# NVIDIA/recsys-examples

Measured on AMD Instinct MI355X. Metric: embedding lookups/sec (DynamicEmb lookup+pool fwd+bwd, steady state), higher is better.
Workload: dtype f32 table rows, f32 accumulate, bf16 pooled output / gradients

## Files before the change

### recsys-examples_amd/csrc/hstu_attn.hip

```cpp
#include "common.h"
#include "../../include/recsys_amd.h"
#include <stdlib.h>
#include <type_traits>


#ifndef HSTU_F16
#define HSTU_F16 0
#endif
#if HSTU_F16
#define HSTU_FN(name) name##_f16
#define HSTU_NS_BEGIN namespace mi355 { inline namespace hstu_f16 {
#define HSTU_NS_END } }
#else
#define HSTU_FN(name) name
#define HSTU_NS_BEGIN namespace mi355 {
#define HSTU_NS_END }
#endif

HSTU_NS_BEGIN

#if HSTU_F16
typedef __attribute__((ext_vector_type(8))) _Float16 bf16x8_t;
#define HSTU_MFMA __builtin_amdgcn_mfma_f32_32x32x16_f16
#else
// ... 1548 lines not shown
  }
  __device__ __forceinline__ void commit_tr(uint16_t* dst, int row0, int L) const {
#pragma unroll
    for (int i = 0; i < PT; ++i) {
      const int ch = threadIdx.x + 256 * i;
      const u32x4_t z = {0u, 0u, 0u, 0u};
      const u32x4_t v = (row0 + ch / (D / 8) < L) ? r[i] : z;
      if (NCH % 256 == 0 || ch < NCH) *reinterpret_cast<u32x4_t*>(dst + (ch / (D / 8)) * TrStride<D>::value + 8 * (ch % (D / 8))) = v;
    }
  }
};

template <int D>
__device__ __forceinline__ void load_own_frags(bf16x8_t (&f)[D / 16], const uint16_t* base, int64_t row_stride, int row, int L, int hi) {
  const uint16_t* p = base + (int64_t)(row < L ? row : L - 1) * row_stride + 8 * hi;
#pragma unroll
  for (int sl = 0; sl < D / 16; ++sl) {
    const u32x4_t t = *reinterpret_cast<const u32x4_t*>(p + 16 * sl);
    f[sl] = __builtin_bit_cast(bf16x8_t, t);
  }
}

struct BwdAttnArgs {
  AttnArgs f;
  const uint16_t* dout; int64_t do_row, do_head;
  uint16_t* dq; uint16_t* dk; uint16_t* dv;
  uint16_t* ds_ws;
  uint16_t* p_ws;
  int ng;
  int bq_kv;
  const int64_t* plan_base;
  const int32_t* plan_chunk;
  int chunk;
  int tri;
  uint16_t* drab; int64_t drab_b, drab_h, drab_r;
  const int2* func_kvis; int64_t func_kvis_h;
  const int4* func_gext;
  int dq_row, dq_head, dk_row, dk_head, dv_row, dv_head;
};
struct XchUnit { int64_t base; int ngb; int tri; };
__device__ __forceinline__ XchUnit xch_unit(const BwdAttnArgs& g, int b, int h, int L) {
  XchUnit u;
  if (g.plan_base) { u.base = g.plan_base[b * g.f.H + h]; u.ngb = (L + 31) >> 5; u.tri = g.tri; }
  else { u.base = ((int64_t)b * g.f.H + h) * g.ng * g.ng; u.ngb = g.ng; u.tri = 0; }
  return u;
}
__device__ __forceinline__ int64_t xch_tile(const XchUnit& u, int kg, int qg) {
  return (u.base + (u.tri ? (int64_t)qg * (qg + 1) / 2 + kg : (int64_t)kg * u.ngb + qg)) * 1024;
}
__device__ __forceinline__ bool xch_absent(const XchUnit& u, int kg, int qg) { return u.tri && kg > qg; }
__device__ __forceinline__ bool xch_other_chunk(const BwdAttnArgs& g, int b, int h) {
  return g.plan_chunk != nullptr && g.plan_chunk[b * g.f.H + h] != g.chunk;
}
constexpr int kPlanMaxU = 4096;
constexpr int kPlanMaxChunks = 2048;
struct PlanView {
  const int64_t* F; int U;
  __device__ __forceinline__ int L(int64_t x) const {
    int lo = 0, hi = U;
    while (lo < hi) { const int mid = (lo + hi + 1) >> 1; if (F[mid] <= x) lo = mid; else hi = mid - 1; }
    return lo;
  }
  __device__ __forceinline__ int next(int s, int64_t c) const {
    const int64_t fs = F[s];
    const int z = L(fs), e = L(fs + c);
    return e > z ? e : (z + 1 < U ? z + 1 : U);
  }
  __device__ __forceinline__ int count(int64_t c) const {
    int n = 0;
    for (int s = 0; s < U; s = next(s, c)) ++n;
    return n > 0 ? n : 1;
  }
};
__global__ void __launch_bounds__(256) hstu_bwd_plan_kernel(const int* cu, int B, int H, int64_t cap_tiles, int tri, int64_t* base,
                                                            int32_t* chunk, int32_t* nchunks_out, int host_chunks, int* host_err) {
  __shared__ int64_t s_F[kPlanMaxU + 1];
  __shared__ int64_t s_part[256];
  __shared__ int s_start[kPlanMaxChunks + 1];
  __shared__ int64_t s_umax;
  __shared__ int s_n;
  __shared__ int64_t s_c;
  if (blockIdx.x != 0) return;
  const int tid = threadIdx.x;
  const int64_t U64 = (int64_t)B * H;
  const bool staged = U64 <= kPlanMaxU;
  if (staged) {
    const int U = (int)U64;
    const int per = (U + 255) / 256, u0 = tid * per < U ? tid * per : U, u1 = u0 + per < U ? u0 + per : U;
    int64_t sum = 0, mx = 1;
    {
      int b = u0 / H, h = u0 - b * H;
      int64_t nd = 0;
      for (int u = u0; u < u1; ++u) {
        if (u == u0 || h == 0) { const int64_t n = (cu[b + 1] - cu[b] + 31) >> 5; nd = tri ? n * (n + 1) / 2 : n * n; }
        s_F[u] = nd;
        sum += nd;
        mx = nd > mx ? nd : mx;
        if (++h == H) { h = 0; ++b; }
      }
    }
    s_part[tid] = sum;
    if (tid == 0) s_umax = 1;
    __syncthreads();
    atomicMax((unsigned long long*)&s_umax, (unsigned long long)mx);
    if (tid < 64) {
      int64_t v[4], run = 0;
// ... 1001 lines not shown
        const uint32_t drop = r0 + 1 < L ? 0u : 0xffffffffu;
        dma16(reinterpret_cast<const char*>(g + (int64_t)rc * row_stride), voff[u] - (rowterm & drop), d0 + u * 1024);
      }
    }
  }
};
typedef Dma64T<8> Dma64;
__device__ __forceinline__ bf16x8_t tr_frag_sw(const uint16_t* tile, int dt, int ks, int lane, int hi) {
  typedef short v4s_t __attribute__((ext_vector_type(4)));
  typedef short v8s_t __attribute__((ext_vector_type(8)));
  typedef __attribute__((address_space(3))) v4s_t* lds_v4s_t;
  const int il = lane & 15, g1 = (lane >> 4) & 1, vq = il >> 2;
  const uint16_t* p0 = tile + (16 * ks + 4 * hi + vq) * 256 + 4 * (il & 1) + 8 * (4 * (dt ^ vq) + 2 * g1 + ((il & 3) >> 1));
  const v4s_t lo4 = __builtin_amdgcn_ds_read_tr16_b64_v4i16((lds_v4s_t)(p0));
  const v4s_t hi4 = __builtin_amdgcn_ds_read_tr16_b64_v4i16((lds_v4s_t)(p0 + 8 * 256));
  const v8s_t r = {lo4.x, lo4.y, lo4.z, lo4.w, hi4.x, hi4.y, hi4.z, hi4.w};
  return __builtin_bit_cast(bf16x8_t, r);
}
template <int BUF>
__device__ __forceinline__ void gemm_x8(f32x16_t (&acc)[8], const uint16_t* ring, const bf16x8_t (&bf)[4], int lane, int hi) {
  constexpr int NB = 8, NVB = HSTU_X8_VBUF;
  const uint16_t* tile = ring + BUF * 64 * 256;
  bf16x8_t fr[NVB][4];
  auto load = [&](int bi) {
#pragma unroll
    for (int u = 0; u < 4; ++u) fr[bi % NVB][u] = tr_frag_sw(tile, 4 * (bi & 1) + u, bi >> 1, lane, hi);
  };
#pragma unroll
  for (int bi = 0; bi < NVB - 1; ++bi) load(bi);
#pragma unroll
  for (int bi = 0; bi < NB; ++bi) {
    if (bi + NVB - 1 < NB) load(bi + NVB - 1);
    __builtin_amdgcn_sched_barrier(0);
#pragma unroll
    for (int u = 0; u < 4; ++u) mfma_a(acc[4 * (bi & 1) + u], fr[bi % NVB][u], bf[bi >> 1]);
    __builtin_amdgcn_sched_barrier(0);
  }
}
template <int D>
__device__ __forceinline__ void store_acc_rows(const f32x16_t (&acc)[D / 32], uint16_t* rowp, int hi) {
#pragma unroll
  for (int dt = 0; dt < D / 32; ++dt)
#pragma unroll
    for (int g4 = 0; g4 < 4; ++g4) {
      uint2 o;
      o.x = pack_bf16(acc[dt][4 * g4 + 0], acc[dt][4 * g4 + 1]);
      o.y = pack_bf16(acc[dt][4 * g4 + 2], acc[dt][4 * g4 + 3]);
      *reinterpret_cast<uint2*>(rowp + 32 * dt + 8 * g4 + 4 * hi) = o;
    }
}

constexpr int kNW8 = 4;

template <int D, bool kFunc = false>
__device__ __forceinline__ void hstu_bwd_v_p8_body(const BwdAttnArgs& g, unsigned bz, unsigned nz) {
  constexpr int NW = kNW8, kBM8 = 32 * NW;
  static_assert(D == 256, "DMA rows of 32 chunks");
  const AttnArgs& a = g.f;
  constexpr int BQ = 64, NT = 2, TILE = BQ * D;
  extern __shared__ __attribute__((aligned(16))) uint16_t smem[];
  const BlockSeq bs = seq_head_of_block(a, bz, nz);
  const int b = bs.b, h = bs.h;
  SeqInfo s;
  s.start = bs.start;
  s.L = bs.end - s.start;
  const int n0 = bs.z * kBM8;
  if (n0 >= s.L || xch_other_chunk(g, b, h)) return;
  const XchUnit xu = xch_unit(g, b, h, s.L);
  s.has_ctx = a.num_contexts != nullptr;
  s.has_tgt = a.num_targets != nullptr;
  s.c = s.has_ctx ? a.num_contexts[b] : 0;
  s.hlen = s.L - (s.has_tgt ? a.num_targets[b] : 0);
  s.wl = a.wl; s.wr = a.wr;
  const int lane = lane_id(), hi = lane >> 5, l31 = lane & 31;
  const int wv = __builtin_amdgcn_readfirstlane((int)(threadIdx.x >> 6));
  const int key0 = n0 + 32 * wv, kj = key0 + l31;
  const bool wave_live = key0 < s.L;
  const uint16_t* dobase = g.dout + (int64_t)s.start * g.do_row + (int64_t)h * g.do_head;
  f32x16_t acc[D / 32];
#pragma unroll
  for (int dt = 0; dt < D / 32; ++dt)
#pragma unroll
    for (int r = 0; r < 16; ++r) acc[dt][r] = 0.f;
  static_assert(kBM8 == kBM, "one key block of the dK pass per workgroup");
  KvSpan sp = kv_span(a, s, n0, g.bq_kv);
  if constexpr (kFunc) sp = kv_span_clip(sp, func_kvis_of(g, s.start, b, h, n0), g.bq_kv);
  const int jump = sp.jump, c_end = sp.c_end, lim = sp.lim;
  const int jump_s = (jump / BQ) * BQ, cend_s = ((c_end + BQ - 1) / BQ) * BQ;
  int i_lim = ((lim + g.bq_kv - 1) / g.bq_kv) * g.bq_kv;
  if (i_lim > s.L) i_lim = s.L;
  auto advance = [&](int i) { i += BQ; return (i >= cend_s && i < jump_s) ? jump_s : i; };
  auto visited = [&](int i) { return i < s.L && kv_visited(sp, (i / g.bq_kv) * g.bq_kv); };
  Dma64T<NW> dma;
  dma.init(wv, lane, g.do_row);
  u32x4_t pn0[NT], pn1[NT];
  auto fetch_p = [&](int i) {
#pragma unroll
    for (int t = 0; t < NT; ++t) {
      const int it = i + 32 * t;
      if (wave_live && visited(it) && !xch_absent(xu, key0 >> 5, it >> 5)) {
        const u32x4_t* tp = reinterpret_cast<const u32x4_t*>(g.p_ws + xch_tile(xu, key0 >> 5, it >> 5)) + 2 * lane;
        pn0[t] = xch_load(tp); pn1[t] = xch_load(tp + 1);
      } else {
        pn0[t] = u32x4_t{0u, 0u, 0u, 0u}; pn1[t] = u32x4_t{0u, 0u, 0u, 0u};
      }
    }
  };
  int i0 = c_end > 0 ? 0 : jump_s;
  if (i0 < i_lim) { dma.issue(dobase, g.do_row, i0, s.L, smem, lane); fetch_p(i0); }
  auto step = [&](auto bufc) {
    constexpr int BUF = decltype(bufc)::value;
    bf16x8_t pf[2 * NT];
    asm volatile("s_waitcnt vmcnt(0)" ::: "memory");
#pragma unroll
    for (int t = 0; t < NT; ++t) { pf[2 * t] = __builtin_bit_cast(bf16x8_t, pn0[t]); pf[2 * t + 1] = __builtin_bit_cast(bf16x8_t, pn1[t]); }
    __syncthreads();
    {
      const int nx = advance(i0);
      if (nx < i_lim) { dma.issue(dobase, g.do_row, nx, s.L, smem + (BUF ^ 1) * TILE, lane); fetch_p(nx); }
    }
    if (wave_live) gemm_x8<BUF>(acc, smem, pf, lane, hi);
    i0 = advance(i0);
  };
  while (i0 < i_lim) {
    step(std::integral_constant<int, 0>{});
    if (i0 >= i_lim) break;
    step(std::integral_constant<int, 1>{});
  }
  asm volatile("s_waitcnt vmcnt(0)" ::: "memory");
  if (kj < s.L) store_acc_rows<D>(acc, g.dv + (int64_t)(s.start + kj) * g.dv_row + (int64_t)h * g.dv_head, hi);
}

template <int D, bool kFunc = false>
__device__ __forceinline__ void hstu_bwd_q_ds8_body(const BwdAttnArgs& g, unsigned bz, unsigned nz) {
  constexpr int NW = kNW8, kBM8 = 32 * NW;
  static_assert(D == 256, "DMA rows of 32 chunks");
  const AttnArgs& a = g.f;
  constexpr int BK = 64, NT = 2, TILE = BK * D;
  extern __shared__ __attribute__((aligned(16))) uint16_t smem[];
  const BlockSeq bs = seq_head_of_block(a, bz, nz);
  const int b = bs.b, h = bs.h;
  SeqInfo s;
  s.start = bs.start;
  s.L = bs.end - s.start;
  const int nblk = (s.L + kBM8 - 1) / kBM8;
  if (bs.z >= nblk || xch_other_chunk(g, b, h)) return;
  const XchUnit xu = xch_unit(g, b, h, s.L);
  const int m0 = row_block_of_rank(bs.z, nblk, a, b) * kBM8;
  s.has_ctx = a.num_contexts != nullptr;
  s.has_tgt = a.num_targets != nullptr;
  s.c = s.has_ctx ? a.num_contexts[b] : 0;
  s.hlen = s.L - (s.has_tgt ? a.num_targets[b] : 0);
  s.wl = a.wl; s.wr = a.wr;
  const int lane = lane_id(), hi = lane >> 5, l31 = lane & 31;
  const int wv = __builtin_amdgcn_readfirstlane((int)(threadIdx.x >> 6));
  uint16_t* dSw = smem + 2 * TILE + NT * 1024 * wv;
  const int qrow0 = m0 + 32 * wv, qi = qrow0 + l31;
  const bool wave_live = qrow0 < s.L;
  int last_row = m0 + kBM8 - 1 < s.L - 1 ? m0 + kBM8 - 1 : s.L - 1;
  int n_end = s.L;
  if (a.causal) { n_end = last_row + 1; if (s.has_ctx && m0 < s.c && s.hlen > n_end) n_end = s.hlen; }
  int w_last = qrow0 + 31 < s.L - 1 ? qrow0 + 31 : s.L - 1;
  int w_end = s.L;
  if (a.causal) { w_end = w_last + 1; if (s.has_ctx && qrow0 < s.c && s.hlen > w_end) w_end = s.hlen; }
  n_end = band_key_end(a, last_row, n_end);
  w_end = band_key_end(a, w_last, w_end);
  int n_beg = band_key_begin(a, m0, BK), w_beg = band_key_begin(a, qrow0, BK);
  const int it_kv = (qrow0 / g.bq_kv) * g.bq_kv;
  int2 vis_all = make_int2(0, 0x7fffffff);
  int gap_a = 0x7fffffff, gap_b = 0x7fffffff;
  int wgap_a = 0x7fffffff, wgap_b = 0x7fffffff;
  if constexpr (kFunc) {
    if (kBM * lane < s.L) vis_all = func_kvis_of(g, s.start, b, h, kBM * lane);
    if (g.func_gext && a.wskip) {
      FuncExt bx{0, 0x7fffffff, 0, 0x7fffffff}, wx = bx;
#pragma unroll
      for (int w = 0; w < NW; ++w) {
        const int row = m0 + 32 * w;
        const int64_t gi = func_gext_index(s.start, b, row);
        FuncExt e{0x7fffffff, 0, 0x7fffffff, 0};
        if (row >= s.L) e = FuncExt{0, 0x7fffffff, 0, 0x7fffffff};
        else if (gi < 4 * g.func_kvis_h) { const int4 t = g.func_gext[(int64_t)(a.func_h ? h : 0) * 4 * g.func_kvis_h + gi]; e = FuncExt{t.y, t.z, t.w, t.x}; }
        bx = func_ext_merge(bx, e);
        if (w == wv) wx = e;
      }
      const int be = func_ext_end(bx), bb = func_ext_begin(bx), we = func_ext_end(wx), wb = func_ext_begin(wx);
      if (be < n_end) n_end = be;
      if (we < w_end) w_end = we;
      if (bb > n_beg) n_beg = bb >= n_end ? n_end : (bb / BK) * BK;
      if (wb > w_beg) w_beg = wb >= 0x7fffff00 ? 0x7fffff00 : (wb / BK) * BK;
      if (bx.lo < bx.hi && bx.lo > bx.f0) {
        const int ga = ((bx.f0 + BK - 1) / BK) * BK, gb = (bx.lo / BK) * BK;
        if (ga < gb) { gap_a = ga; gap_b = gb; }
      }
      if (wx.lo < wx.hi && wx.lo > wx.f0) {
        const int ga = ((wx.f0 + BK - 1) / BK) * BK, gb = (wx.lo / BK) * BK;
        if (ga < gb) { wgap_a = ga; wgap_b = gb; }
      }
      if (n_beg >= gap_a && n_beg < gap_b) n_beg = gap_b;
    }
  }
  auto next_step = [&](int n) { n += BK; if constexpr (kFunc) { if (n >= gap_a && n < gap_b) n = gap_b; } return n; };
  f32x16_t acc[D / 32];
#pragma unroll
  for (int dt = 0; dt < D / 32; ++dt)
#pragma unroll
    for (int r = 0; r < 16; ++r) acc[dt][r] = 0.f;
  const uint16_t* kbase = a.k + (int64_t)s.start * a.k_row + (int64_t)h * a.k_head;
// ... 16 lines not shown
      sp = kv_span_clip(sp, vis, g.bq_kv);
    }
    return kv_visited(sp, it_kv);
  };
  auto fetch_ds = [&](int n) {
#pragma unroll
    for (int t = 0; t < NT; ++t) {
      const int nt = n + 32 * t;
      if (wave_live && nt < w_end && tile_written(nt) && !xch_absent(xu, nt >> 5, qrow0 >> 5)) {
        const u32x4_t* tp = reinterpret_cast<const u32x4_t*>(g.ds_ws + xch_tile(xu, nt >> 5, qrow0 >> 5)) + 2 * lane;
        ds0[t] = xch_load(tp); ds1[t] = xch_load(tp + 1);
      } else {
        ds0[t] = u32x4_t{0u, 0u, 0u, 0u}; ds1[t] = u32x4_t{0u, 0u, 0u, 0u};
      }
    }
  };
  if (n_end > n_beg) { dma.issue(kbase, a.k_row, n_beg, s.L, smem, lane); fetch_ds(n_beg); }
  int n0 = n_beg;
  auto step = [&](auto bufc) {
    constexpr int BUF = decltype(bufc)::value;
    asm volatile("s_waitcnt vmcnt(0)" ::: "memory");
#pragma unroll
    for (int t = 0; t < NT; ++t) {
      *reinterpret_cast<u32x4_t*>(dSw + 1024 * t + 16 * lane) = ds0[t];
      *reinterpret_cast<u32x4_t*>(dSw + 1024 * t + 16 * lane + 8) = ds1[t];
    }
    __syncthreads();
    { const int nx = next_step(n0); if (nx < n_end) { dma.issue(kbase, a.k_row, nx, s.L, smem + (BUF ^ 1) * TILE, lane); fetch_ds(nx); } }
    if (wave_live && n0 < w_end && n0 >= w_beg && !(kFunc && n0 >= wgap_a && n0 < wgap_b)) {
      bf16x8_t sf[2 * NT];
#pragma unroll
      for (int t = 0; t < NT; ++t)
#pragma unroll
        for (int half = 0; half < 2; ++half) {
          const uint16_t* pp = dSw + 1024 * t + tr_lane_off;
          const v4s_t lo4 = __builtin_amdgcn_ds_read_tr16_b64_v4i16((lds_v4s_t)(pp + (8 * (2 * half)) * 16));
          const v4s_t hi4 = __builtin_amdgcn_ds_read_tr16_b64_v4i16((lds_v4s_t)(pp + (8 * (2 * half + 1)) * 16));
          const v8s_t r = {lo4.x, lo4.y, lo4.z, lo4.w, hi4.x, hi4.y, hi4.z, hi4.w};
          sf[2 * t + half] = __builtin_bit_cast(bf16x8_t, r);
        }
      gemm_x8<BUF>(acc, smem, sf, lane, hi);
    }
    n0 = next_step(n0);
  };
  while (n0 < n_end) {
    step(std::integral_constant<int, 0>{});
    if (n0 >= n_end) break;
    step(std::integral_constant<int, 1>{});
  }
  asm volatile("s_waitcnt vmcnt(0)" ::: "memory");
  if (qi < s.L) store_acc_rows<D>(acc, g.dq + (int64_t)(s.start + qi) * g.dq_row + (int64_t)h * g.dq_head, hi);
}

template <int D, bool kFunc = false>
__global__ void __launch_bounds__(64 * kNW8, 2) hstu_bwd_vq8_kernel(BwdAttnArgs g) {
  const unsigned nz = gridDim.z >> 1;
  if (blockIdx.z < nz) hstu_bwd_v_p8_body<D, kFunc>(g, blockIdx.z, nz);
  else hstu_bwd_q_ds8_body<D, kFunc>(g, blockIdx.z - nz, nz);
}

template <int D, bool kFunc = false>
__global__ void __launch_bounds__(512) hstu_bwd_kv_pc_kernel(BwdAttnArgs g) {
  static_assert(D == 256, "DMA rows of 32 chunks");
  const AttnArgs& a = g.f;
  constexpr int BQ = 32, IMG = BQ * D;
  extern __shared__ __attribute__((aligned(16))) uint16_t smem[];
  uint16_t* const Qr = smem;
  uint16_t* const dOr = smem + 2 * IMG;
  uint16_t* const Qt = smem + 4 * IMG;
  uint16_t* const Hs = smem + 6 * IMG;
  int* const Fs = reinterpret_cast<int*>(smem + 6 * IMG + 2 * 4 * 2 * 64 * 8);

  const BlockSeq bs = seq_head_of_block(a);
  const int b = bs.b, h = bs.h;
  SeqInfo s;
  s.start = bs.start;
  s.L = bs.end - s.start;
  const int n0 = bs.z * kBM;
  if (n0 >= s.L || xch_other_chunk(g, b, h)) return;
  const XchUnit xu = xch_unit(g, b, h, s.L);
  s.has_ctx = a.num_contexts != nullptr;
  s.has_tgt = a.num_targets != nullptr;
  s.c = s.has_ctx ? a.num_contexts[b] : 0;
  s.hlen = s.L - (s.has_tgt ? a.num_targets[b] : 0);
  s.wl = a.wl; s.wr = a.wr;
  const int lane = lane_id(), hi = lane >> 5, l31 = lane & 31;
  const int wv = __builtin_amdgcn_readfirstlane((int)(threadIdx.x >> 6));
  const int role = wv >> 2, pw = wv & 3;
  const int key0 = n0 + 32 * pw, kj = key0 + l31;
  const bool wave_live = key0 < s.L;
  const bool plain = !s.has_ctx && !s.has_tgt && s.wl < 0 && s.wr < 0;
  const bool key_in = kj < s.L, key_hist = kj < s.hlen;
  const int key_iend = (s.has_tgt && kj >= s.hlen) ? s.hlen + ((kj - s.hlen) / a.group + 1) * a.group : 0x7fffffff;
  const int ctx_end = s.has_ctx ? s.c : 0;
  const uint16_t* qbase = a.q + (int64_t)s.start * a.q_row + (int64_t)h * a.q_head;
  const uint16_t* dobase = g.dout + (int64_t)s.start * g.do_row + (int64_t)h * g.do_head;
  const float neg_alpha_log2e = -a.alpha * 1.4426950408889634f;
  const float c_p = a.alpha * a.inv_scale, c_ds = a.alpha * a.inv_scale;
  KvSpan span = kv_span(a, s, n0, BQ);
  if constexpr (kFunc) span = kv_span_clip(span, func_kvis_of(g, s.start, b, h, n0), BQ);
  const int jump = span.jump, c_end = span.c_end, i_lim = span.lim;
  auto advance = [&](int i) { i += BQ; return (i >= c_end && i < jump) ? jump : i; };
  const int first = c_end > 0 ? 0 : jump;
#if HSTU_TIMING
  unsigned tsum[7] = {0, 0, 0, 0, 0, 0, 0};
  const unsigned t_start = tick();
  auto t_dump = [&]() {
    const unsigned t_end = tick();
    if (lane == 0) {
      const int blk = ((int)blockIdx.z * gridDim.y + blockIdx.y) * gridDim.x + blockIdx.x;
      unsigned long long* d = g_hstu_dbg + ((size_t)(blk * 8 + wv) % 65536) * 8;
      for (int i = 0; i < 7; ++i) d[i] = tsum[i];
      d[6] |= (unsigned long long)role << 32;
      d[7] = t_end - t_start;
    }
  };
#endif

  const int dr = lane >> 5, dp = lane & 31;
  uint32_t vq_k[4], vdo_k[4], vq_v[4];
#pragma unroll
  for (int u = 0; u < 4; ++u) {
    const int r = 2 * (4 * pw + u) + dr;
    vq_k[u] = (uint32_t)dr * (uint32_t)a.q_row * 2u + 16u * (uint32_t)(dp ^ (r & 15));
    vdo_k[u] = (uint32_t)dr * (uint32_t)g.do_row * 2u + 16u * (uint32_t)(dp ^ (r & 15));
    vq_v[u] = (uint32_t)dr * (uint32_t)a.q_row * 2u + 16u * (uint32_t)(dp ^ ((r & 3) << 2));
  }
  auto issue_img = [&](const uint16_t* gsrc, int64_t row_stride, const uint32_t (&voff)[4], int row0, uint16_t* dst) {
    const uint32_t d0 = __builtin_amdgcn_readfirstlane((uint32_t)(uintptr_t)(lds_void_t)(dst + 8 * pw * D));
    if (row0 + BQ <= s.L) {
      const char* sb = reinterpret_cast<const char*>(gsrc + (int64_t)(row0 + 8 * pw) * row_stride);
      const int64_t step = 2 * row_stride * 2;
#pragma unroll
      for (int u = 0; u < 4; ++u) Dma64::dma16(sb + u * step, voff[u], d0 + u * 1024);
    } else {
      const uint32_t rowterm = (uint32_t)dr * (uint32_t)row_stride * 2u;
#pragma unroll
      for (int u = 0; u < 4; ++u) {
        const int r0 = row0 + 2 * (4 * pw + u);
        const int rc = r0 < s.L ? r0 : s.L - 1;
        const uint32_t drop = r0 + 1 < s.L ? 0u : 0xffffffffu;
        Dma64::dma16(reinterpret_cast<const char*>(gsrc + (int64_t)rc * row_stride), voff[u] - (rowterm & drop), d0 + u * 1024);
      }
    }
  };

  if (role == 0) {
    bf16x8_t kf[D / 16], vf[D / 16];
    load_own_frags<D>(kf, a.k + (int64_t)s.start * a.k_row + (int64_t)h * a.k_head, a.k_row, kj, s.L, hi);
    load_own_frags<D>(vf, a.v + (int64_t)s.start * a.v_row + (int64_t)h * a.v_head, a.v_row, kj, s.L, hi);
    const int kx = l31 & 15;
    int cur = first, prev_valid = 0;
    auto step = [&](auto parc) {
      constexpr int PAR = decltype(parc)::value;
      TICK(t0);
      __syncthreads();
      TICK(t1);
      TACC(0, t0, t1);
      const int i0 = cur;
      const bool have = i0 < i_lim;
      prev_valid = have;
      cur = have ? advance(i0) : i0;
      if (!have || !wave_live) return;
// ... 162 lines not shown
        issue_img(dobase, g.do_row, vdo_k, nxt, dOr + (PAR ^ 1) * IMG);
        fetch_func(nxt);
      }
      issue_img(qbase, a.q_row, vq_v, i0, Qt + PAR * IMG);
    }
    prev_valid = have;
    cur = nxt;
    TICK(t3);
    TACC(2, t2, t3);
    if (!had || !wave_live) return;
    const u32x4_t* hp = reinterpret_cast<const u32x4_t*>(Hs) + (((PAR ^ 1) * 4 + pw) * 2) * 64 + lane;
    bf16x8_t sf[2];
    const u32x4_t y0 = hp[0], y1 = hp[64];
    sf[0] = __builtin_bit_cast(bf16x8_t, y0);
    sf[1] = __builtin_bit_cast(bf16x8_t, y1);
    if (ip < s.L && !xch_absent(xu, key0 >> 5, ip >> 5)) {
      u32x4_t* tq = reinterpret_cast<u32x4_t*>(g.ds_ws + xch_tile(xu, key0 >> 5, ip >> 5)) + 2 * lane;
      xch_store(tq, y0); xch_store(tq + 1, y1);
    }
    const uint16_t* tile = Qt + (PAR ^ 1) * IMG;
    constexpr int NB = 4;
    bf16x8_t fr[2][4];
    auto load = [&](int bi) {
#pragma unroll
      for (int u = 0; u < 4; ++u) fr[bi & 1][u] = tr_frag_sw(tile, 4 * (bi & 1) + u, bi >> 1, lane, hi);
    };
    load(0);
#pragma unroll
    for (int bi = 0; bi < NB; ++bi) {
      if (bi + 1 < NB) load(bi + 1);
      __builtin_amdgcn_sched_barrier(0);
#pragma unroll
      for (int u = 0; u < 4; ++u) mfma_a(acc_dk[4 * (bi & 1) + u], fr[bi & 1][u], sf[bi >> 1]);
      __builtin_amdgcn_sched_barrier(0);
    }
    TICK(t4);
    TACC(5, t3, t4);
#if HSTU_TIMING
    tsum[6] += 1;
#endif
  };
  while (cur < i_lim || prev_valid) {
    step(std::integral_constant<int, 0>{});
    if (!(cur < i_lim || prev_valid)) break;
    step(std::integral_constant<int, 1>{});
  }
  asm volatile("s_waitcnt vmcnt(0)" ::: "memory");
#if HSTU_TIMING
  t_dump();
#endif
  if (kj < s.L) store_acc_rows<D>(acc_dk, g.dk + (int64_t)(s.start + kj) * g.dk_row + (int64_t)h * g.dk_head, hi);
}


static int fwd_hook() {
  static const int v = getenv("MI355_HSTU_FWD") ? atoi(getenv("MI355_HSTU_FWD")) : 0;
  return v;
}

template <auto K, typename Args>
static int launch(dim3 grid, dim3 block, size_t smem, hipStream_t stream, const Args& args) {
  static bool attr_set = false;
  if (!attr_set) {
    const hipError_t e = hipFuncSetAttribute(reinterpret_cast<const void*>(K), hipFuncAttributeMaxDynamicSharedMemorySize, (int)smem);
    if (e != hipSuccess) { mi355_set_error(hipGetErrorString(e)); return MI355_ELAUNCH; }
    attr_set = true;
  }
  hipLaunchKernelGGL(K, grid, block, smem, stream, args);
  return MI355_OK;
}
static int launched(int failed) {
  if (failed) return MI355_ELAUNCH;
  MI355_LAUNCH_CHECK();
  return MI355_OK;
}

template <int D, int BQ, int MODE, bool kPre, bool kXP = false, bool kRab = false, bool kDq = false, bool kBoth = false>
static int launch_bwd_kv(const BwdAttnArgs& g, dim3 grid, hipStream_t stream) {
  constexpr bool kDV = MODE != 2, kDK = MODE != 1;
  const size_t timg = (size_t)BQ * TrStride<D>::value;
  const size_t smem = (size_t)(BQ * (D + 8) + (kDK ? BQ * (D + 8) + timg : 0) + (kDV ? timg : 0)) * sizeof(uint16_t);
  return launch<hstu_bwd_kv_kernel<D, BQ, MODE, kPre, kXP, kRab, kDq, kBoth>>(grid, dim3(256), smem, stream, g);
}
template <int D, int BK, bool kPre, bool kRab = false, bool kDq = false, bool kBoth = false>
static int launch_bwd_q(const BwdAttnArgs& g, dim3 grid, hipStream_t stream) {
  const size_t smem_q = (size_t)(2 * BK * (D + 8) + BK * TrStride<D>::value) * sizeof(uint16_t);
  return launch<hstu_bwd_q_kernel<D, BK, kPre, kRab, kDq, kBoth>>(grid, dim3(256), smem_q, stream, g);
}

template <int D>
static int launch_bwd_v_p(const BwdAttnArgs& g, dim3 grid, hipStream_t stream) {
  const size_t smem = (size_t)(HSTU_XSTEP * TrStride<D>::value) * sizeof(uint16_t);
  return launch<hstu_bwd_v_p_kernel<D>>(grid, dim3(256), smem, stream, g);
}

template <int D>
static int launch_bwd_q_ds(const BwdAttnArgs& g, dim3 grid, hipStream_t stream) {
  const size_t smem = (size_t)(HSTU_XSTEP * TrStride<D>::value + 4 * (HSTU_XSTEP / 32) * 1024) * sizeof(uint16_t);
  return launch<hstu_bwd_q_ds_kernel<D>>(grid, dim3(256), smem, stream, g);
}

template <bool kFunc>
static int launch_bwd_pc_x8(const BwdAttnArgs& g, dim3 grid, int B, int max_seqlen, hipStream_t stream) {
  const size_t smem_pc = (size_t)(6 * 32 * 256 + 2 * 4 * 2 * 64 * 8) * sizeof(uint16_t) + (kFunc ? 2 * 192 * sizeof(int) : 0);
  const size_t smem = (size_t)(2 * 64 * 256 + kNW8 * 2 * 1024) * sizeof(uint16_t);
  const int nblk = (max_seqlen + 32 * kNW8 - 1) / (32 * kNW8);
  return launched(launch<hstu_bwd_kv_pc_kernel<256, kFunc>>(grid, dim3(512), smem_pc, stream, g) ||
                  launch<hstu_bwd_vq8_kernel<256, kFunc>>(dim3(g.f.H, B, 2 * nblk), dim3(64 * kNW8), smem, stream, g));
}

template <int D>
static int launch_bwd(BwdAttnArgs g, int B, int max_seqlen, hipStream_t stream) {
  dim3 grid(g.f.H, B, (max_seqlen + kBM - 1) / kBM);
  if constexpr (D == 256) {
    if (g.f.func && !g.f.rab && g.f.n_func <= 5 && g.p_ws && g.ds_ws) {
      g.bq_kv = 32;
      return launch_bwd_pc_x8<true>(g, grid, B, max_seqlen, stream);
    }
  }
  if (g.f.rab && g.f.func) {
    g.ds_ws = g.p_ws = nullptr;
    g.bq_kv = 64;
    if constexpr (D >= 128)
      return launched(launch_bwd_kv<D, 64, 1, false, false, true, false, true>(g, grid, stream) ||
                      launch_bwd_kv<D, 32, 2, false, false, true, false, true>(g, grid, stream) ||
                      launch_bwd_q<D, D >= 256 ? 32 : 64, false, true, false, true>(g, grid, stream));
    else
      return launched(launch_bwd_kv<D, 64, 0, false, false, true, false, true>(g, grid, stream) ||
                      launch_bwd_q<D, 64, false, true, false, true>(g, grid, stream));
  }
  if (g.f.rab || g.f.func) {
    g.ds_ws = g.p_ws = nullptr;
    g.bq_kv = 64;
    if constexpr (D >= 128)
      return launched(launch_bwd_kv<D, 64, 1, false, false, true>(g, grid, stream) ||
                      launch_bwd_kv<D, 32, 2, false, false, true>(g, grid, stream) ||
                      launch_bwd_q<D, D >= 256 ? 32 : 64, false, true>(g, grid, stream));
    else
      return launched(launch_bwd_kv<D, 64, 0, false, false, true>(g, grid, stream) || launch_bwd_q<D, 64, false, true>(g, grid, stream));
  }
  if constexpr (D >= 256) {
    if (g.p_ws) {
      g.bq_kv = 32;
      return launch_bwd_pc_x8<false>(g, grid, B, max_seqlen, stream);
    }
    g.bq_kv = 64;
    return launched(launch_bwd_kv<D, 64, 1, true>(g, grid, stream) || launch_bwd_kv<D, 64, 2, false>(g, grid, stream) ||
                    (g.ds_ws ? launch_bwd_q_ds<D>(g, grid, stream) : launch_bwd_q<D, 32, true>(g, grid, stream)));
  } else if constexpr (D >= 128) {
    g.bq_kv = 32;
    if (g.p_ws)
      return launched(launch_bwd_kv<D, 32, 2, false, true>(g, grid, stream) || launch_bwd_v_p<D>(g, grid, stream) ||
                      launch_bwd_q_ds<D>(g, grid, stream));
    return launched(launch_bwd_kv<D, 64, 1, false>(g, grid, stream) || launch_bwd_kv<D, 32, 2, false>(g, grid, stream) ||
                    (g.ds_ws ? launch_bwd_q_ds<D>(g, grid, stream) : launch_bwd_q<D, 64, false>(g, grid, stream)));
  } else {
    g.bq_kv = 64;
    g.p_ws = nullptr;
    return launched(launch_bwd_kv<D, 64, 0, false>(g, grid, stream) ||
                    (g.ds_ws ? launch_bwd_q_ds<D>(g, grid, stream) : launch_bwd_q<D, 64, false>(g, grid, stream)));
  }
}

template <int D, bool kRab>
static int launch_bwd_dq(BwdAttnArgs g, int B, int max_q, int max_k, hipStream_t stream) {
  const dim3 gk(g.f.H, B, (max_k + kBM - 1) / kBM), gq(g.f.H, B, (max_q + kBM - 1) / kBM);
  g.ds_ws = g.p_ws = nullptr;
  g.bq_kv = 64;
  constexpr bool kPre = D >= 256 && !kRab;
  int failed;
  if constexpr (D >= 128)
    failed = launch_bwd_kv<D, 64, 1, kPre, false, kRab, true>(g, gk, stream) ||
             launch_bwd_kv<D, (D >= 256 && !kRab) ? 64 : 32, 2, false, false, kRab, true>(g, gk, stream);
  else
    failed = launch_bwd_kv<D, 64, 0, false, false, kRab, true>(g, gk, stream);
  return launched(failed || (max_q > 0 && launch_bwd_q<D, D >= 256 ? 32 : 64, kPre, kRab, true>(g, gq, stream)));
}

template <int D>
static int launch_fwd_pc(const AttnArgs& a, int B, int max_seqlen, hipStream_t stream, bool dense_batch) {
  const size_t smem = (size_t)(4 * kBN * D + 2 * 4 * 4 * 64 * 8) * sizeof(uint16_t);
  const int hook = fwd_hook();
  const bool paired = hook == 2 || hook == 4 || dense_batch;
  const bool q2 = hook == 1 || hook == 2 || (hook != 3 && hook != 4 && max_seqlen > 1024) || a.func;
  const int nblk = (max_seqlen + kBM - 1) / kBM;
  const bool win = a.wl >= 0 || a.wr >= 0;
  const dim3 grid(a.H, B, paired ? (nblk + 1) / 2 : nblk), block(512);
  if (q2) {
    if (a.func)
      return launched(paired ? launch<hstu_fwd_q2_kernel<D, true, true, true>>(grid, block, smem, stream, a)
                             : launch<hstu_fwd_q2_kernel<D, true, false, true>>(grid, block, smem, stream, a));
    if (paired)
      return launched(win ? launch<hstu_fwd_q2_kernel<D, true, true>>(grid, block, smem, stream, a)
                          : launch<hstu_fwd_q2_kernel<D, false, true>>(grid, block, smem, stream, a));
    return launched(win ? launch<hstu_fwd_q2_kernel<D, true, false>>(grid, block, smem, stream, a)
                        : launch<hstu_fwd_q2_kernel<D, false, false>>(grid, block, smem, stream, a));
  }
// ... 183 lines not shown
  if (batch == 0 || max_seqlen == 0) return MI355_OK;
  if (int* ew = plan_err_word()) {
    if (*ew) {
      *ew = 0;
      mi355_set_error("an earlier hstu backward planned more exchange chunks than were launched (token hint of another batch?): "
                      "its gradients are incomplete");
      return MI355_EINVAL;
    }
  }
  BwdAttnArgs g{};
  fill(g, c);
  const AttnArgs& a = g.f;
  if (a.func && c.func_ws && a.wskip) {
    const int64_t nfh = a.func_h ? num_heads : 1;
    const int64_t slots = c.func_ws_bytes / 72 / nfh;
    if (slots > 0 && ((uintptr_t)c.func_ws & 15) == 0) {
      const size_t sm = 4 * (size_t)((max_seqlen + 31) / 32) * sizeof(int);
      int4* gext = (int4*)c.func_ws;
      int2* kvis = (int2*)(gext + nfh * 4 * slots);
      hipLaunchKernelGGL(hstu_func_kvis_kernel, dim3((unsigned)batch, (unsigned)nfh), dim3(256), sm, c.stream, a, (int)nfh, kvis, slots, gext);
      g.func_kvis = kvis; g.func_kvis_h = slots; g.func_gext = gext;
    }
  }
  int nchunks = 1;
  {
    const int64_t need = mi355_hstu_attn_bwd_ds_bytes(batch, num_heads, head_dim, max_seqlen);
    const int64_t regions = xch_regions(head_dim), units = batch * num_heads, hdr = xch_plan_header(units);
    const int64_t udense = (int64_t)g.ng * g.ng;
    g.tri = (c.causal && !c.num_contexts && c.wl < 0 && c.wr < 0 && !c.rab && !c.func) ? 1 : 0;
    const int64_t umax = xch_unit_tiles(g.ng, g.tri);
    if (need > 0 && c.ws && c.ws_bytes >= need && ((uintptr_t)c.ws & 15) == 0) {
      g.ds_ws = (uint16_t*)c.ws;
      const int64_t one = batch * num_heads * udense * 2048;
      if (need >= 2 * one && head_dim >= 128) g.p_ws = (uint16_t*)((uint8_t*)c.ws + one);
    } else if (need > 0 && c.ws && ((uintptr_t)c.ws & 255) == 0 && !c.rab && (!c.func || (head_dim == 256 && c.n_func <= 5)) &&
               c.ws_bytes > hdr && (c.ws_bytes - hdr) / regions / 2048 >= 2 * umax) {
      const int64_t cap_tiles = (c.ws_bytes - hdr) / regions / 2048;
      uint8_t* w = (uint8_t*)c.ws;
      int64_t* base = (int64_t*)w;
      int32_t* chunk = (int32_t*)(w + (units * 8 + 255) / 256 * 256);
      int32_t* nch = (int32_t*)(w + hdr - 256);
      g.plan_base = base; g.plan_chunk = chunk;
      g.ds_ws = (uint16_t*)(w + hdr);
      if (regions == 2) g.p_ws = (uint16_t*)(w + hdr + cap_tiles * 2048);
      const int64_t bound = xch_tiles_bound(batch, num_heads, g.ng, c.tokens_hint, g.tri);
      nchunks = (int)((bound + (cap_tiles - umax)) / (cap_tiles - umax + 1));
      if (bound <= cap_tiles) nchunks = 1;
      if (nchunks < 1) nchunks = 1;
      if (nchunks > units) nchunks = (int)units;
      hipLaunchKernelGGL(hstu_bwd_plan_kernel, dim3(1), dim3(256), 0, c.stream, c.cu_seqlens_q, (int)batch, (int)num_heads, cap_tiles, g.tri,
                         base, chunk, nch, nchunks, plan_err_word());
    }
  }
  for (int ch = 0; ch < nchunks; ++ch) {
    g.chunk = ch;
    int rc;
    switch (head_dim) {
      case 32: rc = launch_bwd<32>(g, (int)batch, (int)max_seqlen, c.stream); break;
      case 64: rc = launch_bwd<64>(g, (int)batch, (int)max_seqlen, c.stream); break;
      case 128: rc = launch_bwd<128>(g, (int)batch, (int)max_seqlen, c.stream); break;
      default: rc = launch_bwd<256>(g, (int)batch, (int)max_seqlen, c.stream); break;
    }
    if (rc != MI355_OK) return rc;
  }
  return MI355_OK;
}

static int hstu_backward_dq(const HstuCall& c) {
  if (c.batch == 0 || c.max_seqlen_k == 0) return MI355_OK;
  BwdAttnArgs g{};
  fill(g, c);
  g.f.rot = 0; g.f.colmajor = 0; g.f.max_len = (int)c.max_seqlen_k;
  const int B = (int)c.batch, mq = (int)c.max_seqlen_q, mk = (int)c.max_seqlen_k;
  if (c.rab) {
    switch (c.head_dim) {
      case 32: return launch_bwd_dq<32, true>(g, B, mq, mk, c.stream);
      case 64: return launch_bwd_dq<64, true>(g, B, mq, mk, c.stream);
      case 128: return launch_bwd_dq<128, true>(g, B, mq, mk, c.stream);
      default: return launch_bwd_dq<256, true>(g, B, mq, mk, c.stream);
    }
  }
  switch (c.head_dim) {
    case 32: return launch_bwd_dq<32, false>(g, B, mq, mk, c.stream);
    case 64: return launch_bwd_dq<64, false>(g, B, mq, mk, c.stream);
    case 128: return launch_bwd_dq<128, false>(g, B, mq, mk, c.stream);
    default: return launch_bwd_dq<256, false>(g, B, mq, mk, c.stream);
  }
}

extern "C" {
#if HSTU_TIMING && !HSTU_F16
int mi355_hstu_dbg_dump(void* out, int64_t bytes) {
  return (int)hipMemcpyFromSymbol(out, HIP_SYMBOL(mi355::g_hstu_dbg), (size_t)bytes);
}
#endif

int HSTU_FN(mi355_hstu_attn_fwd)(const void* q, const void* k, const void* v, void* out, int64_t q_row_stride,
                        int64_t k_row_stride, int64_t v_row_stride, int64_t o_row_stride, int64_t q_head_stride,
                        int64_t k_head_stride, int64_t v_head_stride, int64_t o_head_stride, const int32_t* cu_seqlens,
                        int64_t batch, int64_t num_heads, int64_t head_dim, int64_t max_seqlen,
                        const int32_t* num_contexts, const int32_t* num_targets, int64_t target_group_size, int causal,
                        float alpha, float scaling_seqlen, hipStream_t stream) {
  HstuCall c = forward_call(out, q, k, v, q_row_stride, k_row_stride, v_row_stride, o_row_stride, q_head_stride, k_head_stride,
                            v_head_stride, o_head_stride, cu_seqlens, nullptr, batch, num_heads, head_dim, max_seqlen, max_seqlen,
                            alpha, scaling_seqlen, stream);
  c.num_contexts = num_contexts; c.num_targets = num_targets; c.group = target_group_size; c.causal = causal;
  return hstu_forward(c);
}

int HSTU_FN(mi355_hstu_attn_fwd_kv)(const void* q, const void* k, const void* v, void* out, int64_t q_row_stride,
                           int64_t k_row_stride, int64_t v_row_stride, int64_t o_row_stride, int64_t q_head_stride,
                           int64_t k_head_stride, int64_t v_head_stride, int64_t o_head_stride, const int32_t* cu_seqlens_q,
                           const int32_t* cu_seqlens_k, int64_t batch, int64_t num_heads, int64_t head_dim,
                           int64_t max_seqlen_q, const int32_t* num_contexts, const int32_t* num_targets,
// ... 333 lines not shown
```

Baseline: 3.047 billion.

## Pair causal row blocks per workgroup in D=256 HSTU backward for load balance

When all sequences are full length and the grid is small compared with the CU count, the D=256 backward kernels launch half as many z-blocks. Each workgroup then handles block z and its mirror block (nblk-1-z) in two passes, which balances the triangular causal work. This targets tail imbalance and idle CUs in small grids. It costs a barrier between passes, less parallelism, and a tid re-materialisation trick. The metric is embedding lookups, so this attention path may not be exercised at all.

```diff
diff --git a/recsys-examples_amd/csrc/hstu_attn.hip b/recsys-examples_amd/csrc/hstu_attn.hip
--- a/recsys-examples_amd/csrc/hstu_attn.hip
+++ b/recsys-examples_amd/csrc/hstu_attn.hip
@@ -1624,6 +1624,8 @@
 __device__ __forceinline__ bool xch_other_chunk(const BwdAttnArgs& g, int b, int h) {
   return g.plan_chunk != nullptr && g.plan_chunk[b * g.f.H + h] != g.chunk;
 }
+__device__ __forceinline__ int bwd_pair_rank(const AttnArgs& a, int z) { return (a.max_len + kBM - 1) / kBM - 1 - z; }
+__device__ __forceinline__ int tid_fresh() { int t = (int)threadIdx.x; asm volatile("" : "+v"(t)); return t; }
 constexpr int kPlanMaxU = 4096;
 constexpr int kPlanMaxChunks = 2048;
 struct PlanView {
@@ -2731,14 +2733,15 @@
 
 constexpr int kNW8 = 4;
 
-template <int D, bool kFunc = false>
-__device__ __forceinline__ void hstu_bwd_v_p8_body(const BwdAttnArgs& g, unsigned bz, unsigned nz) {
+template <int D, bool kFunc, bool kPair>
+__device__ __forceinline__ void hstu_bwd_v_p8_body(const BwdAttnArgs& g, unsigned bz, unsigned nz, int pass) {
   constexpr int NW = kNW8, kBM8 = 32 * NW;
   static_assert(D == 256, "DMA rows of 32 chunks");
   const AttnArgs& a = g.f;
   constexpr int BQ = 64, NT = 2, TILE = BQ * D;
   extern __shared__ __attribute__((aligned(16))) uint16_t smem[];
-  const BlockSeq bs = seq_head_of_block(a, bz, nz);
+  BlockSeq bs = seq_head_of_block(a, bz, nz);
+  if (kPair && pass) bs.z = bwd_pair_rank(a, bs.z);
   const int b = bs.b, h = bs.h;
   SeqInfo s;
   s.start = bs.start;
@@ -2751,8 +2754,8 @@
   s.c = s.has_ctx ? a.num_contexts[b] : 0;
   s.hlen = s.L - (s.has_tgt ? a.num_targets[b] : 0);
   s.wl = a.wl; s.wr = a.wr;
-  const int lane = lane_id(), hi = lane >> 5, l31 = lane & 31;
-  const int wv = __builtin_amdgcn_readfirstlane((int)(threadIdx.x >> 6));
+  const int tid = kPair ? tid_fresh() : (int)threadIdx.x, lane = kPair ? tid & 63 : lane_id(), hi = lane >> 5, l31 = lane & 31;
+  const int wv = __builtin_amdgcn_readfirstlane(kPair ? tid >> 6 : (int)(threadIdx.x >> 6));
   const int key0 = n0 + 32 * wv, kj = key0 + l31;
   const bool wave_live = key0 < s.L;
   const uint16_t* dobase = g.dout + (int64_t)s.start * g.do_row + (int64_t)h * g.do_head;
@@ -2810,14 +2813,15 @@
   if (kj < s.L) store_acc_rows<D>(acc, g.dv + (int64_t)(s.start + kj) * g.dv_row + (int64_t)h * g.dv_head, hi);
 }
 
-template <int D, bool kFunc = false>
-__device__ __forceinline__ void hstu_bwd_q_ds8_body(const BwdAttnArgs& g, unsigned bz, unsigned nz) {
+template <int D, bool kFunc, bool kPair>
+__device__ __forceinline__ void hstu_bwd_q_ds8_body(const BwdAttnArgs& g, unsigned bz, unsigned nz, int pass) {
   constexpr int NW = kNW8, kBM8 = 32 * NW;
   static_assert(D == 256, "DMA rows of 32 chunks");
   const AttnArgs& a = g.f;
   constexpr int BK = 64, NT = 2, TILE = BK * D;
   extern __shared__ __attribute__((aligned(16))) uint16_t smem[];
-  const BlockSeq bs = seq_head_of_block(a, bz, nz);
+  BlockSeq bs = seq_head_of_block(a, bz, nz);
+  if (kPair && pass) bs.z = bwd_pair_rank(a, bs.z);
   const int b = bs.b, h = bs.h;
   SeqInfo s;
   s.start = bs.start;
@@ -2831,8 +2835,8 @@
   s.c = s.has_ctx ? a.num_contexts[b] : 0;
   s.hlen = s.L - (s.has_tgt ? a.num_targets[b] : 0);
   s.wl = a.wl; s.wr = a.wr;
-  const int lane = lane_id(), hi = lane >> 5, l31 = lane & 31;
-  const int wv = __builtin_amdgcn_readfirstlane((int)(threadIdx.x >> 6));
+  const int tid = kPair ? tid_fresh() : (int)threadIdx.x, lane = kPair ? tid & 63 : lane_id(), hi = lane >> 5, l31 = lane & 31;
+  const int wv = __builtin_amdgcn_readfirstlane(kPair ? tid >> 6 : (int)(threadIdx.x >> 6));
   uint16_t* dSw = smem + 2 * TILE + NT * 1024 * wv;
   const int qrow0 = m0 + 32 * wv, qi = qrow0 + l31;
   const bool wave_live = qrow0 < s.L;
@@ -2955,15 +2959,28 @@
   if (qi < s.L) store_acc_rows<D>(acc, g.dq + (int64_t)(s.start + qi) * g.dq_row + (int64_t)h * g.dq_head, hi);
 }
 
-template <int D, bool kFunc = false>
+template <int D, bool kFunc = false, bool kPair = false>
 __global__ void __launch_bounds__(64 * kNW8, 2) hstu_bwd_vq8_kernel(BwdAttnArgs g) {
   const unsigned nz = gridDim.z >> 1;
-  if (blockIdx.z < nz) hstu_bwd_v_p8_body<D, kFunc>(g, blockIdx.z, nz);
-  else hstu_bwd_q_ds8_body<D, kFunc>(g, blockIdx.z - nz, nz);
-}
-
-template <int D, bool kFunc = false>
-__global__ void __launch_bounds__(512) hstu_bwd_kv_pc_kernel(BwdAttnArgs g) {
+  if constexpr (!kPair) {
+    if (blockIdx.z < nz) hstu_bwd_v_p8_body<D, kFunc, false>(g, blockIdx.z, nz, 0);
+    else hstu_bwd_q_ds8_body<D, kFunc, false>(g, blockIdx.z - nz, nz, 0);
+  } else {
+    const unsigned bz = blockIdx.z < nz ? blockIdx.z : blockIdx.z - nz;
+    for (int pass = 0; pass < 2; ++pass) {
+      if (pass) {
+        const int z = seq_head_of_block(g.f, bz, nz).z;
+        if (bwd_pair_rank(g.f, z) <= z) break;
+        __syncthreads();
+      }
+      if (blockIdx.z < nz) hstu_bwd_v_p8_body<D, kFunc, true>(g, bz, nz, pass);
+      else hstu_bwd_q_ds8_body<D, kFunc, true>(g, bz, nz, pass);
+    }
+  }
+}
+
+template <int D, bool kFunc, bool kPair>
+__device__ __forceinline__ void hstu_bwd_kv_pc_block(const BwdAttnArgs& g, int pass) {
   static_assert(D == 256, "DMA rows of 32 chunks");
   const AttnArgs& a = g.f;
   constexpr int BQ = 32, IMG = BQ * D;
@@ -2974,7 +2991,8 @@
   uint16_t* const Hs = smem + 6 * IMG;
   int* const Fs = reinterpret_cast<int*>(smem + 6 * IMG + 2 * 4 * 2 * 64 * 8);
 
-  const BlockSeq bs = seq_head_of_block(a);
+  BlockSeq bs = seq_head_of_block(a);
+  if (kPair && pass) bs.z = bwd_pair_rank(a, bs.z);
   const int b = bs.b, h = bs.h;
   SeqInfo s;
   s.start = bs.start;
@@ -2987,8 +3005,8 @@
   s.c = s.has_ctx ? a.num_contexts[b] : 0;
   s.hlen = s.L - (s.has_tgt ? a.num_targets[b] : 0);
   s.wl = a.wl; s.wr = a.wr;
-  const int lane = lane_id(), hi = lane >> 5, l31 = lane & 31;
-  const int wv = __builtin_amdgcn_readfirstlane((int)(threadIdx.x >> 6));
+  const int tid = kPair ? tid_fresh() : (int)threadIdx.x, lane = kPair ? tid & 63 : lane_id(), hi = lane >> 5, l31 = lane & 31;
+  const int wv = __builtin_amdgcn_readfirstlane(kPair ? tid >> 6 : (int)(threadIdx.x >> 6));
   const int role = wv >> 2, pw = wv & 3;
   const int key0 = n0 + 32 * pw, kj = key0 + l31;
   const bool wave_live = key0 < s.L;
@@ -3011,7 +3029,7 @@
   auto t_dump = [&]() {
     const unsigned t_end = tick();
     if (lane == 0) {
-      const int blk = ((int)blockIdx.z * gridDim.y + blockIdx.y) * gridDim.x + blockIdx.x;
+      const int blk = (bs.z * gridDim.y + b) * gridDim.x + h;
       unsigned long long* d = g_hstu_dbg + ((size_t)(blk * 8 + wv) % 65536) * 8;
       for (int i = 0; i < 7; ++i) d[i] = tsum[i];
       d[6] |= (unsigned long long)role << 32;
@@ -3280,6 +3298,22 @@
   if (kj < s.L) store_acc_rows<D>(acc_dk, g.dk + (int64_t)(s.start + kj) * g.dk_row + (int64_t)h * g.dk_head, hi);
 }
 
+template <int D, bool kFunc = false, bool kPair = false>
+__global__ void __launch_bounds__(512) hstu_bwd_kv_pc_kernel(BwdAttnArgs g) {
+  if constexpr (!kPair) {
+    hstu_bwd_kv_pc_block<D, kFunc, false>(g, 0);
+  } else {
+    for (int pass = 0; pass < 2; ++pass) {
+      if (pass) {
+        const int z = seq_head_of_block(g.f).z;
+        if (bwd_pair_rank(g.f, z) <= z) break;
+        __syncthreads();
+      }
+      hstu_bwd_kv_pc_block<D, kFunc, true>(g, pass);
+    }
+  }
+}
+
 
 static int fwd_hook() {
   static const int v = getenv("MI355_HSTU_FWD") ? atoi(getenv("MI355_HSTU_FWD")) : 0;
@@ -3329,21 +3363,29 @@
 }
 
 template <bool kFunc>
-static int launch_bwd_pc_x8(const BwdAttnArgs& g, dim3 grid, int B, int max_seqlen, hipStream_t stream) {
+static int launch_bwd_pc_x8(const BwdAttnArgs& g, dim3 grid, int B, int max_seqlen, bool pair, hipStream_t stream) {
   const size_t smem_pc = (size_t)(6 * 32 * 256 + 2 * 4 * 2 * 64 * 8) * sizeof(uint16_t) + (kFunc ? 2 * 192 * sizeof(int) : 0);
   const size_t smem = (size_t)(2 * 64 * 256 + kNW8 * 2 * 1024) * sizeof(uint16_t);
-  const int nblk = (max_seqlen + 32 * kNW8 - 1) / (32 * kNW8);
+  static_assert(32 * kNW8 == kBM, "one block size, one pairing rule (bwd_pair_rank) for the three passes");
+  const int nblk = (max_seqlen + kBM - 1) / kBM;
+  constexpr int kCUs = 256;
+  if (pair && (int64_t)g.f.H * B * nblk <= 2 * kCUs) {
+    const int nz = (nblk + 1) / 2;
+    grid.z = nz;
+    return launched(launch<hstu_bwd_kv_pc_kernel<256, kFunc, true>>(grid, dim3(512), smem_pc, stream, g) ||
+                    launch<hstu_bwd_vq8_kernel<256, kFunc, true>>(dim3(g.f.H, B, 2 * nz), dim3(64 * kNW8), smem, stream, g));
+  }
   return launched(launch<hstu_bwd_kv_pc_kernel<256, kFunc>>(grid, dim3(512), smem_pc, stream, g) ||
                   launch<hstu_bwd_vq8_kernel<256, kFunc>>(dim3(g.f.H, B, 2 * nblk), dim3(64 * kNW8), smem, stream, g));
 }
 
 template <int D>
-static int launch_bwd(BwdAttnArgs g, int B, int max_seqlen, hipStream_t stream) {
+static int launch_bwd(BwdAttnArgs g, int B, int max_seqlen, hipStream_t stream, bool pair = false) {
   dim3 grid(g.f.H, B, (max_seqlen + kBM - 1) / kBM);
   if constexpr (D == 256) {
     if (g.f.func && !g.f.rab && g.f.n_func <= 5 && g.p_ws && g.ds_ws) {
       g.bq_kv = 32;
-      return launch_bwd_pc_x8<true>(g, grid, B, max_seqlen, stream);
+      return launch_bwd_pc_x8<true>(g, grid, B, max_seqlen, pair, stream);
     }
   }
   if (g.f.rab && g.f.func) {
@@ -3370,7 +3412,7 @@
   if constexpr (D >= 256) {
     if (g.p_ws) {
       g.bq_kv = 32;
-      return launch_bwd_pc_x8<false>(g, grid, B, max_seqlen, stream);
+      return launch_bwd_pc_x8<false>(g, grid, B, max_seqlen, pair, stream);
     }
     g.bq_kv = 64;
     return launched(launch_bwd_kv<D, 64, 1, true>(g, grid, stream) || launch_bwd_kv<D, 64, 2, false>(g, grid, stream) ||
@@ -3660,6 +3702,7 @@
                          base, chunk, nch, nchunks, plan_err_word());
     }
   }
+  const bool pair = c.tokens_hint == batch * max_seqlen;
   for (int ch = 0; ch < nchunks; ++ch) {
     g.chunk = ch;
     int rc;
@@ -3667,7 +3710,7 @@
       case 32: rc = launch_bwd<32>(g, (int)batch, (int)max_seqlen, c.stream); break;
       case 64: rc = launch_bwd<64>(g, (int)batch, (int)max_seqlen, c.stream); break;
       case 128: rc = launch_bwd<128>(g, (int)batch, (int)max_seqlen, c.stream); break;
-      default: rc = launch_bwd<256>(g, (int)batch, (int)max_seqlen, c.stream); break;
+      default: rc = launch_bwd<256>(g, (int)batch, (int)max_seqlen, c.stream, pair); break;
     }
     if (rc != MI355_OK) return rc;
   }
```

After: 2.979 billion. -2.2%, worse.
